# crowsonkb/style_transfer

Hardware: AMD Instinct MI355X
Metric: tile-iterations/sec, VGG-19 2048px/1024-tile (fwd+bwd, Gram/content losses, regularizers, Adam step) (higher is better)
Workload: dtype f32 (fp16x2-split MFMA, fp32 accumulate)

## Files before the change

### style_transfer_amd/csrc/common.h

```cpp
#pragma once

#include <hip/hip_runtime.h>

#include <vector>

#include <cstdarg>
#include <cstdio>
#include <functional>
#include <string>

#include "stx.h"

namespace stx {

constexpr float kEps = 1.1920928955078125e-07f;

void set_error(const char *fmt, ...);

const char *sw_env(const char *name);
void sw_reread();

#define STX_HIP(call)                                                                       \
    do {                                                                                    \
        hipError_t err__ = (call);                                                          \
// ... 120 lines not shown
    bool pin_mask = false;
#ifdef STX_EXPERIMENT_BF3
    const void *x_split = nullptr;
#endif
};

enum class ConvFamily { Direct, Wino2, H2 };

struct ConvConfig {
    ConvFamily family;
    int id;
    int bm;
    int kc;
    int pr, pc;
    int threads;
    size_t lds_bytes;
};

ConvConfig conv_pick_config(int ksize, int K, int M, int H, int W);
ConvConfig conv_config_by_id(int id);
bool direct_takes_inject(const ConvConfig &cfg);
int conv_num_workgroups(const ConvConfig &cfg, int M, int H, int W);
size_t conv_packed_floats(const ConvConfig &cfg, int K, int M, int ksize);
int conv_pack_weights(hipStream_t s, const float *w_caffe, int Mo, int Ko, int ksize,
                      int transpose_flip, const ConvConfig &cfg, float *packed);
int conv_launch(hipStream_t s, const ConvConfig &cfg, const ConvProblem &p, bool packed_weights);
int direct_splitk_factor(const ConvConfig &cfg, const ConvProblem &p, bool packed_weights);

int splitk_reduce_launch(hipStream_t s, const ConvProblem &p, int ksplit);
int splitk_reduce_items_launch(hipStream_t s, const ConvProblem &p, const ConvConfig &cfg, int slices,
                               int item_base, int items);
__host__ __device__ inline void wino2_item_tiles(int lt, int m_tiles, int n_patches, int &pt, int &mt) {
    pt = lt / m_tiles;
    mt = lt - pt * m_tiles;
    if (m_tiles == 8 && (n_patches & 7) == 0) {
        const int g = lt >> 5, r = lt & 31;
        mt = (g & 1) * 4 + (r & 3);
        pt = (g >> 1) * 8 + (r >> 2);
    }
}

struct WinoArgs {
    const float *x;
    const float *w;
    float *y;
    const float *bias;
    const float *mask;
    int K, M, H, W;
    int n_chunks, tiles_x, tiles_y, m_tiles, ksplit;
    int w_tile_stride;
    int x_bytes, w_bytes;
    int relu;
    ConvInject inj;
    float *pool_out;
    int pool_mode;
    unsigned char *pool_codes;
    int skip_y = 0;
    unsigned char *out_codes = nullptr;
    unsigned char *in_codes = nullptr;
    const unsigned char *mask_codes = nullptr;
    long long *clock_out = nullptr;
    int item_base = 0;
    const unsigned *x_amax = nullptr;
    unsigned *y_amax = nullptr;
    const unsigned char *pin_codes = nullptr;
    int pin_mode = 0, pin_mask = 0;
#ifdef STX_EXPERIMENT_BF3
    int vp_rows = 0, vp_tp = 0;
#endif
};

bool conv_first_usable(int K, int M, int ksize);
int conv_first_workgroups(int H, int W);
int conv_first_launch(hipStream_t s, const float *x, const float *w_caffe, const float *bias, float *y,
                      int K, int H, int W, int relu, float *gram_partials, unsigned *y_amax = nullptr);

ConvConfig wino2_config(int geometry = 0);
int wino2_pick_geometry(int H, int W);
size_t wino2_packed_floats(int K, int M);
int wino2_pack_weights(hipStream_t s, const float *w_caffe, int Mo, int Ko, int transpose_flip,
                       float *packed);
int wino2_launch(hipStream_t s, const ConvConfig &cfg, const ConvProblem &p, int ksplit);
bool wino2_fuses_pool(const ConvProblem &p);
bool wino2_uses_relu_codes(const ConvProblem &p, int ksplit);
bool wino2_writes_out_codes(const ConvConfig &cfg, const ConvProblem &p);
int wino2_splitk_factor(const ConvConfig &cfg, const ConvProblem &p);
struct Wino2Tail { int items, slices; };
Wino2Tail wino2_tail_split(const ConvConfig &cfg, const ConvProblem &p);
int wino2_max_slices(const ConvConfig &cfg, const ConvProblem &p);

constexpr int kAmaxSlots = 64;
ConvConfig h2_config(int mb, int pb = 1);
ConvConfig h2_pick_config(const ConvProblem &p);
bool h2_usable(const ConvProblem &p);
size_t h2_packed_floats(int K, int M);
int h2_pack_weights(hipStream_t s, const float *w_caffe, int Mo, int Ko, int transpose_flip, float *packed);
int h2_launch(hipStream_t s, const ConvConfig &cfg, const ConvProblem &p, int ksplit);
int h2_splitk_factor(const ConvConfig &cfg, const ConvProblem &p);
bool h2_fuses_pool(const ConvProblem &p);
bool h2_takes_pooled_input(const ConvConfig &cfg, const ConvProblem &p);
int absmax_launch(hipStream_t s, const float *x, size_t n, unsigned *slots);

size_t conv_small_packed_floats(int K);
int conv_small_pack(hipStream_t s, const float *w_caffe, int Mo, int Ko, int transpose_flip,
                    float *packed);
int conv_small_launch(hipStream_t s, const float *x, const float *packed, float *y,
                      const float *mask, int K, int M, int H, int W);

bool conv_h2_enabled();
struct ConvTuner { int device; hipStream_t stream; hipEvent_t ev0, ev1; std::function<int(const ConvConfig &, const float **)> bank; };
int conv_choose(const ConvProblem &p, bool winograd, const ConvTuner *tuner, ConvConfig *out);
struct ConvBank { int key; size_t floats; std::function<int(hipStream_t, const float *w_caffe, float *packed)> pack; };
ConvBank conv_bank(const ConvConfig &cfg, int dir, int Mo, int Ko, int ksize);
ConvBank conv_small_bank(int Mo, int Ko);
int conv_dispatch(hipStream_t s, const ConvConfig &cfg, const ConvProblem &p, double *flop_algorithmic,
                  double *flop_issued);
int conv_splitk_factor(const ConvConfig &cfg, const ConvProblem &p);
size_t conv_splitk_floats(const ConvConfig &cfg, const ConvProblem &p);
bool conv_takes_clock(const ConvConfig &cfg);
bool conv_fuses_pool(const ConvConfig &cfg, const ConvProblem &p);
bool conv_writes_pool_codes(const ConvConfig &cfg);
bool conv_reads_x_amax(const ConvConfig &cfg);
bool conv_leaves_y_amax(const ConvConfig &cfg);
bool conv_takes_inject(const ConvConfig &cfg);
bool conv_takes_pooled_input(const ConvConfig &cfg, const ConvProblem &p);
bool conv_uses_relu_codes(const ConvConfig &cfg, const ConvProblem &p, int ksplit);
bool conv_writes_out_codes(const ConvConfig &cfg, const ConvProblem &p, int ksplit);

int pool_forward_launch(hipStream_t s, const float *x, int C, int H, int W, int mode, float *y,
                        unsigned char *codes = nullptr);
int pool_backward_codes_launch(hipStream_t s, const float *dy, const unsigned char *codes, int C,
                               int H, int W, int mode, bool relu_mask, float *dx);
int pool_backward_launch(hipStream_t s, const float *dy, const float *x, int C, int H, int W,
                         int mode, bool relu_mask, float *dx);

struct GramPlan {
    int C, HW, splits, tiles;
    int parts;
    size_t partial_floats;
};
GramPlan gram_plan(int C, int HW);
bool gram_h2_usable(const float *feat, int C, int HW);
int gram_partials_launch(hipStream_t s, const float *feat, const GramPlan &plan, float *partials,
                         const unsigned *f_amax = nullptr);
int gram_finish_blocks(const GramPlan &plan);
int gram_finish_launch(hipStream_t s, const float *partials, const GramPlan &plan, float *gram_out,
                       const float *target, float *dsym, float *sumsq, unsigned short *pieces = nullptr,
                       const unsigned *f_amax = nullptr, float *block_out = nullptr);

size_t symm_pieces_elems(int C);
int symm_num_workgroups(int C, int HW);
bool symm_bf3_usable(const float *feat, const float *out, int C, int HW);
bool symm_h2_usable(const float *feat, const float *out, int C, int HW);
int symm_h2_launch(hipStream_t s, const float *feat, const float *dsym, const unsigned *d_amax, int n_damax,
                   const unsigned *f_amax, float *out, float *partials, int C, int HW);
int symm_bf3_launch(hipStream_t s, const float *feat, const float *dsym, unsigned short *pieces,
                    bool pieces_ready, float *out, float *partials, int C, int HW);

#ifdef __HIPCC__
__device__ __forceinline__ int content_origin_y(const ContentWindow &w) { return w.oy - w.sy; }
__device__ __forceinline__ int content_origin_x(const ContentWindow &w) { return w.ox - w.sx; }
__device__ __forceinline__ size_t content_index(const ContentWindow &w, int c, int y, int x) {
    int yy = (content_origin_y(w) + y) % w.ch;
    int xx = (content_origin_x(w) + x) % w.cw;
    if (yy < 0) yy += w.ch;
    if (xx < 0) xx += w.cw;
    return ((size_t)c * w.ch + yy) * w.cw + xx;
}
#endif

struct SumJob {
    const float *src;
    int n;
    float *dst;
};
int sum_jobs_launch(hipStream_t s, const SumJob *jobs, int n_jobs);
int content_sums_launch(hipStream_t s, const float *feat, const float *content,
                        const ContentWindow &win, float *sums , std::vector<SumJob> *defer = nullptr);
int inject_style_launch(hipStream_t s, float *diff, const float *sgrad, size_t n,
                        const float *abs_sum, float coef, bool accumulate, unsigned *y_amax = nullptr);
int inject_content_launch(hipStream_t s, float *diff, const float *feat, const float *content,
                          const ContentWindow &win, const float *sums, float coef, bool accumulate,
                          unsigned *y_amax = nullptr);
int relu_inplace_launch(hipStream_t s, float *x, size_t n);
int sum_partials_launch(hipStream_t s, const float *partials, int n, float *out);
int sum_partials2_launch(hipStream_t s, const float *a, int na, float *out_a, const float *b, int nb,
                         float *out_b);

constexpr int kMaskParts = 1024;
constexpr int kMaskSgradParts = 2048;
int mask_map_launch(hipStream_t s, const float *mask, int H, int W, int scale, float *out);
int mask_apply_launch(hipStream_t s, const float *feat, const float *map, const ContentWindow &win, float *fm,
                      float *m2_partials, int *n_parts);
int mask_target_launch(hipStream_t s, const float *gs, int C, const float *m2_partials, int n_parts, int HW,
                       float *out, float *a_out);
int mask_sgrad_launch(hipStream_t s, float *sgrad, const float *map, const ContentWindow &win, const float *a,
                      float *partials, int *n_parts);

constexpr int kContentMaskParts = 1024;
int content_mask_mean_launch(hipStream_t s, const float *map, const ContentWindow &win, float *a_out);
int content_mask_term_launch(hipStream_t s, const float *feat, const float *content, const float *map,
                             const ContentWindow &win, const float *a, float *sgrad, float *partials,
                             int *n_parts);

constexpr int kStatSlice = 16384;
constexpr float kStatEps = 1e-5f;
int stat_slices(int HW);
size_t stat_scratch_floats(int C, int HW);
int stat_partials_launch(hipStream_t s, const float *feat, int C, int HW, float *partials);
int stat_finish_launch(hipStream_t s, const float *partials, int C, int HW, const float *MU, const float *SD,
                       float *table, float *e_out, float *mean_out, float *sd_out);
int stat_grad_launch(hipStream_t s, const float *feat, int C, int HW, const float *table, float *sgrad,
                     float *abs_partials, int *n_parts);

int cut_tile_launch(hipStream_t s, const float *img, int H, int W, int rx, int ry, int y0, int x0,
                    int th, int tw, float *tile);
int put_tile_launch(hipStream_t s, float *grad, int H, int W, int rx, int ry, int y0, int x0,
                    int th, int tw, const float *tile);
int place_window_launch(hipStream_t s, float *dst, int dh, int dw, int y0, int x0, const float *src,
                        int C, int h, int w);
int roll_add_launch(hipStream_t s, float *acc, const float *src, int C, int h, int w, int sx, int sy,
                    float alpha, bool init);
int resample_launch(hipStream_t s, int axis, const float *src, int C, int H, int W, float *dst,
                    int OH, int OW, const int *bounds, const double *k, int ksize, int clamp);
int finish_partials_launch(hipStream_t s, const float *partials, int n, double *out_dev);
int finish_partials_n_launch(hipStream_t s, const float *partials, int n, int nv, double *out_dev);
int regularizers_launch(hipStream_t s, const float *img, float *grad, int H, int W,
                        const float mean[3], float tv_scale, float tv_power, float p_scale,
                        float p_power, const float *aux, float aux_scale, int aux_rx, int aux_ry,
                        double *loss_terms , float *scratch, size_t scratch_floats);

int swt_padded_side(int H, int W);
int swt_haar_launch(hipStream_t s, const float *img, float *grad, int H, int W, int rx, int ry,
                    float scale, float power, double *loss_term, float *scratch,
                    size_t scratch_floats);
void swt_levels_scratch(int H, int W, size_t *tmp_floats, size_t *partial_floats);
int swt_haar_levels_launch(hipStream_t s, const float *img, float *grad, int H, int W, int levels,
                           int rx, int ry, float scale, float power, double *loss_term, float *tmp,
                           float *partials);
void swt_daub_table(int order, int levels, int N, std::vector<float> *taps, int *hl);
int swt_table_launch(hipStream_t s, const float *img, float *grad, int H, int W, const float *table,
                     int ntaps, int hl, int rx, int ry, float scale, float power,
                     double *loss_term, float *tmp, float *partials);

constexpr int kLapMaxPools = 4;
struct LapLevels {
    int n;
    int lp[kLapMaxPools], hp[kLapMaxPools], wp[kLapMaxPools], off[kLapMaxPools];
};
size_t lap_levels(int H, int W, int n_pools, const int *pools, LapLevels *lv);
size_t lap_scratch_floats(size_t map_floats);
int lap_target_launch(hipStream_t s, const float *content, int H, int W, const LapLevels &lv,
                      float *target, float *scratch);
int lap_launch(hipStream_t s, const float *img, float *grad, int H, int W, const LapLevels &lv,
               size_t map_floats, const float *coefs, const float *target, double *loss_terms,
               float *scratch);

int adam_launch(hipStream_t s, float *params, const float *grad, float *g1, float *g2, float *p1,
                float *avg, size_t n, double lr, double b1, double b2, double bp1, double c1,
                double c2, double cp);
int dot_launch(hipStream_t s, const float *x, const float *y, size_t n, double *out_dev,
               float *scratch, size_t scratch_floats);
int abs_sum_launch(hipStream_t s, const float *x, size_t n, double *out_dev, float *scratch,
                   size_t scratch_floats);
int axpy_launch(hipStream_t s, float a, const float *x, float *y, size_t n);
int scale_launch(hipStream_t s, float a, float *x, size_t n);
int axpy_dev_launch(hipStream_t s, double c1, const double *a, double da, double c2, const double *b,
                    double db, const float *x, float *y, size_t n);
int scale_dev_launch(hipStream_t s, double c, const double *den, double den_div, float *x, size_t n);
int axpy_dot_dev_launch(hipStream_t s, double c1, const double *a, double da, double c2, const double *b,
                        double db, double c_s, const double *den_s, double div_s, const float *x,
                        const float *src, float *y, const float *z, size_t n, double *out_dev, float *scratch,
                        size_t scratch_floats);
int lbfgs_pair_launch(hipStream_t s, const float *g_new, float *g_old, const float *sv, float *y, size_t n,
                      double *out_dev2, float *scratch, size_t scratch_floats);
int scale2_axpy_launch(hipStream_t s, float c1, float c2, float *sv, float *params, size_t n);
int step_stats_launch(hipStream_t s, const float *avg, float *old, int H, int W,
                      double *out_dev , float *scratch, size_t scratch_floats);
int to_u8_launch(hipStream_t s, const float *img, int H, int W, const float mean[3], uint8_t *out);
int to_u8_luma_launch(hipStream_t s, const float *img, const float *content, int H, int W,
                      const float mean[3], uint8_t *out);
int color_stats_launch(hipStream_t s, const float *img, int H, int W, double *out_dev ,
                       float *scratch, size_t scratch_floats);
int color_affine_launch(hipStream_t s, const float *src, float *dst, int H, int W, const double A[9],
                        const double b[3], const float mean[3]);

}
```

### style_transfer_amd/csrc/symm.hip

```cpp

#include <algorithm>
#include <cstdlib>
#include <cstring>

#include "bf16x3.h"
#include "common.h"
#include "f16x2.h"

#ifndef STX_SYMM_SKIP
#define STX_SYMM_SKIP 0
#endif

namespace stx {

namespace {

constexpr int kSM = 64;
constexpr int kSN = 256;
#ifndef STX_SYMM_KSK
#define STX_SYMM_KSK 32
#endif
constexpr int kSK = STX_SYMM_KSK;
constexpr int kSPC = kSK / 16;
constexpr int kSegs = kSK / 8;
// ... 213 lines not shown
    const __amdgpu_buffer_rsrc_t rd =
        __builtin_amdgcn_make_buffer_rsrc(const_cast<float *>(D), 0, (unsigned)(C * C) * 4u, 0x00020000);
    unsigned voff[2];
#pragma unroll
    for (int j = 0; j < 2; ++j) {
        const int px = px0 + j * 32 + l31;
        voff[j] = px < HW ? (unsigned)((g * 8) * HW + px) * 4u : kOob;
    }
    const unsigned HW4 = (unsigned)HW * 4u;
    const int n_steps = Cp / 16, n_chunks = Cp / kSK;

    unsigned dvoff[kHDLoads], ddst[kHDLoads];
    int dcol[kHDLoads];
#pragma unroll
    for (int n = 0; n < kHDLoads; ++n) {
        const int e = tid + 256 * n;
        const int row = e / (kSK / 4), seg = e - row * (kSK / 4);
        dcol[n] = seg * 4;
        dvoff[n] = m0 + row < C ? (unsigned)((m0 + row) * C + seg * 4) * 4u : kOob;
        ddst[n] = (unsigned)(row * kRowBytes + seg * 8);
    }
    u32x4y dreg[kHDLoads];
    auto d_load = [&](int chunk) {
        const unsigned so = (unsigned)__builtin_amdgcn_readfirstlane(chunk * kSK * 4);
#pragma unroll
        for (int n = 0; n < kHDLoads; ++n)
            dreg[n] = __builtin_amdgcn_raw_buffer_load_b128(rd, dcol[n] + chunk * kSK < C ? dvoff[n] : kOob, so, 0);
    };

    float raw[kRing][2][8];
    auto f_load = [&](int step, int slot_) {
        const int k0 = __builtin_amdgcn_readfirstlane(step * 16);
        const int left = C - k0 < 16 ? C - k0 : 16;
        const __amdgpu_buffer_rsrc_t rk =
            BIG ? __builtin_amdgcn_make_buffer_rsrc(const_cast<float *>(F) + (size_t)k0 * (size_t)HW, 0,
                                                    (left > 0 ? left : 0) * HW * 4, 0x00020000)
                : rf;
#pragma unroll
        for (int j = 0; j < 2; ++j)
#pragma unroll
            for (int e = 0; e < 8; ++e)
                raw[slot_][j][e] = __builtin_bit_cast(
                    float, __builtin_amdgcn_raw_buffer_load_b32(
                               rk, voff[j], BIG ? (unsigned)e * HW4 : (unsigned)min(k0 + e, C) * HW4, 0));
    };

    f32x16h acc[2][2];
#pragma unroll
    for (int i = 0; i < 2; ++i)
#pragma unroll
        for (int j = 0; j < 2; ++j)
#pragma unroll
            for (int r = 0; r < 16; ++r) acc[i][j][r] = 0.f;

    d_load(0);
#pragma unroll
    for (int r = 0; r < kRing - 1; ++r)
        if (r < n_steps) f_load(r, r);

    const int ef = h2_scale_exp(amax_of_slots(f_amax, kAmaxSlots));
    unsigned dm = 0;
    for (int i = tid; i < n_damax; i += 256) dm = max(dm, d_amax[i]);
#pragma unroll
    for (int off = 32; off > 0; off >>= 1) dm = max(dm, (unsigned)__shfl_xor((int)dm, off, 64));
    if (lane == 0) wave_max[wave] = dm;
    __syncthreads();
    dm = max(max(wave_max[0], wave_max[1]), max(wave_max[2], wave_max[3]));
    const int ed = __builtin_amdgcn_readfirstlane(h2_scale_exp(dm));
    const float sf = pow2f(ef), sd = pow2f(ed);

    auto d_store = [&](int buf) {
#pragma unroll
        for (int n = 0; n < kHDLoads; ++n) {
            unsigned h[2], l[2];
            const unsigned d0 = dreg[n].x, d1 = dreg[n].y, d2 = dreg[n].z, d3 = dreg[n].w;
            split2_f16_quad(__builtin_bit_cast(float, d0), __builtin_bit_cast(float, d1),
                            __builtin_bit_cast(float, d2), __builtin_bit_cast(float, d3), sd, h, l);
            typedef unsigned u32x2s __attribute__((ext_vector_type(2)));
            unsigned char *q = lds + buf * kHChunkBytes + ddst[n];
            *reinterpret_cast<u32x2s *>(q) = (u32x2s){h[0], h[1]};
            *reinterpret_cast<u32x2s *>(q + kPieceBytes) = (u32x2s){l[0], l[1]};
        }
    };
    d_store(0);
    if (n_chunks > 1) d_load(1);
    __syncthreads();

    const unsigned a_off = (unsigned)(l31 * kRowBytes + g * 16);
    auto do_step = [&](int slot_, int buf, int s_in_chunk) {
        f16x8h bh[2], bl[2], ah[2], al[2];
#pragma unroll
        for (int j = 0; j < 2; ++j) split2_f16(raw[slot_][j], sf, bh[j], bl[j]);
        const unsigned char *base = lds + buf * kHChunkBytes + a_off + s_in_chunk * 32;
#pragma unroll
        for (int i = 0; i < 2; ++i) {
            ah[i] = *reinterpret_cast<const f16x8h *>(base + i * 32 * kRowBytes);
            al[i] = *reinterpret_cast<const f16x8h *>(base + kPieceBytes + i * 32 * kRowBytes);
        }
#pragma unroll
        for (int i = 0; i < 2; ++i)
#pragma unroll
            for (int j = 0; j < 2; ++j) acc[i][j] = mfma_split3(ah[i], al[i], bh[j], bl[j], acc[i][j]);
    };

    int step = 0;
    auto advance = [&](int slot_) {
        const int chunk = step / kSPC, s_in = step % kSPC, buf = chunk & 1;
        if (step + kRing - 1 < n_steps) f_load(step + kRing - 1, (slot_ + kRing - 1) % kRing);
        do_step(slot_, buf, s_in);
        if (s_in == kSPC - 1) {
            if (chunk + 1 < n_chunks) d_store(buf ^ 1);
            if (chunk + 2 < n_chunks) d_load(chunk + 2);
            __syncthreads();
        }
        ++step;
    };
    while (step < n_steps) {
#pragma unroll
        for (int r = 0; r < kRing; ++r)
            if (step < n_steps) advance(r);
    }

    const float ud = pow2f(-ed), uf = pow2f(-ef);
    float asum = 0.f;
#pragma unroll
    for (int i = 0; i < 2; ++i)
#pragma unroll
        for (int r = 0; r < 16; ++r) {
            const int row = m0 + i * 32 + (r & 3) + 8 * (r >> 2) + 4 * g;
            const int row0 = min(__builtin_amdgcn_readfirstlane(m0 + i * 32 + (r & 3) + 8 * (r >> 2)), C);
            const unsigned so = BIG ? 0u : (unsigned)row0 * HW4;
            const int rows_left = C - row0 < 5 ? C - row0 : 5;
            const __amdgpu_buffer_rsrc_t rrow =
                BIG ? __builtin_amdgcn_make_buffer_rsrc(S + (size_t)row0 * (size_t)HW, 0,
                                                        (rows_left > 0 ? rows_left : 0) * HW * 4, 0x00020000)
                    : rs;
#pragma unroll
            for (int j = 0; j < 2; ++j) {
                const int px = px0 + j * 32 + l31;
                const bool ok = row < C && px < HW;
                const float v = (acc[i][j][r] * ud) * uf;
                asum += ok ? fabsf(v) : 0.f;
                const unsigned vo = ok ? (unsigned)((4 * g) * HW + px) * 4u : kOob;
                __builtin_amdgcn_raw_buffer_store_b32(__builtin_bit_cast(unsigned, v), rrow, vo, so, 0);
            }
        }
#pragma unroll
    for (int off = 32; off > 0; off >>= 1) asum += __shfl_down(asum, off, 64);
    if (lane == 0) wave_sum[wave] = asum;
    __syncthreads();
    if (tid == 0) partials[blockIdx.x] = ((wave_sum[0] + wave_sum[1]) + wave_sum[2]) + wave_sum[3];
}

__global__ void symm_split_kernel(const float *__restrict__ dsym, int C, int Cp,
                                  unsigned short *__restrict__ pieces) {
    const int idx = blockIdx.x * blockDim.x + threadIdx.x;
    if (idx >= Cp * Cp) return;
    const int i = idx / Cp, j = idx - i * Cp;
    unsigned short s1 = 0, s2 = 0, s3 = 0;
    if (i < C && j < C) split3_bf16_scalar(dsym[i * C + j], s1, s2, s3);
    pieces[idx] = s1;
    pieces[(size_t)Cp * Cp + idx] = s2;
    pieces[2 * (size_t)Cp * Cp + idx] = s3;
}

int symm_num_workgroups(int C, int HW) { return ceil_div(C, kSM) * ceil_div(HW, kSN); }

bool symm_bf3_usable(const float *feat, const float *out, int C, int HW) {
    const char *env = sw_env("STX_SYMM");
    if (env && !strcmp(env, "fp32")) return false;
    return 64.0 * (double)HW < 2147483648.0 &&
           ((reinterpret_cast<uintptr_t>(feat) | reinterpret_cast<uintptr_t>(out)) & 3) == 0;
}

int symm_bf3_launch(hipStream_t s, const float *feat, const float *dsym, unsigned short *pieces,
                    bool pieces_ready, float *out, float *partials, int C, int HW) {
    const int Cp = ceil_div(C, kSM) * kSM;
    if (!pieces_ready || Cp != C) {
        symm_split_kernel<<<ceil_div(Cp * Cp, 256), 256, 0, s>>>(dsym, C, Cp, pieces);
        STX_CHECK_LAUNCH();
    }
    const int m_tiles = Cp / kSM;
    const double bytes = 4.0 * C * (double)HW;
    const char *force_big = sw_env("STX_WINO_BIG");
    if (bytes >= 2147483648.0 || (force_big && atoi(force_big) == 1))
        symm_bf3_kernel<true><<<symm_num_workgroups(C, HW), 256, 0, s>>>(feat, pieces, out, partials, C, Cp,
                                                                       HW, 0u, m_tiles);
    else
        symm_bf3_kernel<false><<<symm_num_workgroups(C, HW), 256, 0, s>>>(feat, pieces, out, partials, C, Cp,
                                                                        HW, (unsigned)bytes, m_tiles);
    STX_CHECK_LAUNCH();
    return STX_OK;
}

bool symm_h2_usable(const float *feat, const float *out, int C, int HW) {
    const char *env = sw_env("STX_SYMM");
    if (env && (!strcmp(env, "fp32") || !strcmp(env, "bf3"))) return false;
    return C % 4 == 0 && symm_bf3_usable(feat, out, C, HW);
}

int symm_h2_launch(hipStream_t s, const float *feat, const float *dsym, const unsigned *d_amax, int n_damax,
                   const unsigned *f_amax, float *out, float *partials, int C, int HW) {
    const int Cp = ceil_div(C, kSM) * kSM;
    const int m_tiles = Cp / kSM;
    const double bytes = 4.0 * C * (double)HW;
    const char *force_big = sw_env("STX_WINO_BIG");
    if (bytes >= 2147483648.0 || (force_big && atoi(force_big) == 1))
        symm_h2_kernel<true><<<symm_num_workgroups(C, HW), 256, 0, s>>>(feat, dsym, d_amax, n_damax, f_amax, out,
                                                                      partials, C, Cp, HW, 0u, m_tiles);
    else
        symm_h2_kernel<false><<<symm_num_workgroups(C, HW), 256, 0, s>>>(feat, dsym, d_amax, n_damax, f_amax, out,
                                                                       partials, C, Cp, HW, (unsigned)bytes, m_tiles);
    STX_CHECK_LAUNCH();
    return STX_OK;
}

}
```

### style_transfer_amd/csrc/tile_path.cpp

```cpp

#include <algorithm>
#include <cmath>
#include <cstdlib>
#include <deque>

#include "engine.h"

namespace stx {

ConvProblem conv_fwd_problem(const float *x, float *y, const float *bias, int Cin, int Cout, int H, int W,
                             int ks, int relu) {
    ConvProblem p{};
    p.x = x;
    p.y = y;
    p.bias = bias;
    p.K = Cin;
    p.M = Cout;
    p.H = H;
    p.W = W;
    p.ksize = ks;
    p.relu = relu;
    p.epilogue = kEpiForward;
    return p;
}
// ... 206 lines not shown
        p.pool_out = pt.data.f();
        p.pool_mode = pool->pool_mode;
        pt.codes_valid = false;
        pt.amax_data = -1;
        if (conv_fuses_pool(cfg, p)) {
            *pooled = true;
            pt.amax_data = t.amax_data;
            if (conv_writes_pool_codes(cfg) && e->pool_codes) {
                STX_TRY(pt.codes.ensure(pt.count() + 4));
                p.pool_codes = static_cast<unsigned char *>(pt.codes.ptr);
                pt.codes_valid = true;
                p.skip_y = plan.top_unobserved;
            }
        } else {
            p.pool_out = nullptr;
        }
    }
    t.relu_codes_valid = false;
    if (plan.relu_codes && t.relu && plan.conv_reader && conv_h2_enabled()) {
        const size_t bytes = (size_t)t.channels * ((t.h + 1) / 2) * ((t.w + 1) / 2);
        STX_TRY(t.relu_codes.ensure(bytes));
        p.out_codes = static_cast<unsigned char *>(t.relu_codes.ptr);
        t.relu_codes_valid = conv_writes_out_codes(cfg, p, conv_splitk_factor(cfg, p));
        if (!t.relu_codes_valid) p.out_codes = nullptr;
    }
    ProfScope scope(e, "fwd " + L.name, direct);
    return launch_conv(e, cfg, p);
}

static ConvProblem conv_backward_shape(stx_engine *e, int li) {
    const Layer &L = e->layers[li];
    const Blob &b = e->blobs[L.bottom_blob];
    const ConvParams &cp = e->sh->conv[li];
    return conv_bwd_problem(nullptr, nullptr, nullptr, cp.cout, cp.cin, b.h, b.w, cp.ks);
}

static bool conv_backward_takes_pooled(stx_engine *e, int li) {
    const char *env = sw_env("STX_POOL_BWD_FUSE");
    if (env && atoi(env) == 0) return false;
    const ConvProblem p = conv_backward_shape(e, li);
    ConvConfig cfg;
    return p.ksize == 3 && p.M > 4 && conv_choose(p, e->winograd, nullptr, &cfg) == STX_OK &&
           conv_takes_pooled_input(cfg, p);
}

static int run_conv_backward(stx_engine *e, int li, const ConvInject *inj, bool *fused, const Layer *pooled) {
    const Layer &L = e->layers[li];
    Blob &b = e->blobs[L.bottom_blob];
    const Blob &t = e->blobs[L.top_blob];
    const ConvParams &cp = e->sh->conv[li];
    ConvProblem p = conv_backward_shape(e, li);
    p.x = t.diff.f();
    p.y = b.diff.f();
    p.mask = b.relu ? b.data.f() : nullptr;
    p.mask_codes = b.relu && b.relu_codes_valid ? static_cast<const unsigned char *>(b.relu_codes.ptr) : nullptr;
    p.wants_codes = b.relu && b.relu_codes_wanted;
    if (cp.ks == 3 && cp.cin <= 4) {
        if (fused) *fused = false;
        const float *packed = nullptr;
        STX_TRY(get_bank(e, li, conv_small_bank(cp.cout, cp.cin), &packed));
        const double direct = conv_flops(cp.cout, cp.cin, b.h, b.w, cp.ks);
        ProfScope scope(e, "bwd " + L.name, direct);
        e->flop_algorithmic += direct;
        e->flop_issued += direct * 4.0 / p.M;
        return conv_small_launch(e->stream, p.x, packed, p.y, p.mask, p.K, p.M, p.H, p.W);
    }
    ConvConfig cfg;
    STX_TRY(choose_conv(e, li, 1, p, &cfg));
    const bool can_fuse = inj && conv_takes_inject(cfg);
    if (fused) *fused = can_fuse;
    if (can_fuse) p.inject = *inj;
    b.amax_diff = -1;
    if (pooled) {
        const Blob &pt = e->blobs[pooled->top_blob];
        if (!conv_takes_pooled_input(cfg, p) || !pt.codes_valid) {
            set_error("run_conv_backward: %s cannot take the gradient of %s pooled", L.name.c_str(), pt.name.c_str());
            return STX_ERR_UNSUPPORTED;
        }
        p.x = pt.diff.f();
        p.pin_codes = static_cast<const unsigned char *>(pt.codes.ptr);
        p.pin_mode = pooled->pool_mode;
        p.pin_mask = t.relu;
        STX_TRY(amax_for(e, pooled->top_blob, true, &p.x_amax));
    } else if (conv_reads_x_amax(cfg)) {
        STX_TRY(amax_for(e, L.top_blob, true, &p.x_amax));
    }
    if (conv_leaves_y_amax(cfg)) {
        p.y_amax = e->amax_slots(L.bottom_blob, true);
        b.amax_diff = L.bottom_blob;
    }
    STX_TRY(get_packed(e, li, 1, cfg, &p.w));
    STX_TRY(attach_splitk(e, cfg, p));
    ProfScope scope(e, "bwd " + L.name, conv_flops(cp.cout, cp.cin, b.h, b.w, cp.ks));
    return launch_conv(e, cfg, p);
}

static size_t style_term_scratch_floats(int C, int HW) {
    return 2 * (size_t)ceil_div(C * C, 64) + (size_t)symm_num_workgroups(C, HW) + 64;
}

int launch_style_terms(stx_engine *e, hipStream_t stream, const float *feat, int C, int h, int w,
                       const float *target, float *sgrad, float *sc, const std::string &name,
                       const unsigned *f_amax, float *term_scratch, std::vector<SumJob> *defer) {
    const int HW = h * w;
    const bool fused = e->first_gram_valid && e->first_gram_blob >= 0 &&
                       feat == e->blobs[e->first_gram_blob].data.f() && C == 64;
    GramPlan plan = gram_plan(C, HW);
    if (fused) {
        plan.splits = e->first_gram_parts;
        plan.tiles = 1;
        plan.parts = 1;
        plan.partial_floats = (size_t)plan.splits * 64 * 64;
    }
    const int fin_blocks = gram_finish_blocks(plan);
    float *const partials = fused ? e->first_gram.f() : nullptr;
    if (!fused) STX_TRY(e->gram_partials.ensure((plan.partial_floats + 2 * fin_blocks) * sizeof(float)));
    STX_TRY(e->dsym.ensure((size_t)C * C * sizeof(float)));
    const bool gram_h2 = !fused && gram_h2_usable(feat, C, HW);
    const bool symm_h2 = symm_h2_usable(feat, sgrad, C, HW);
    const bool bf3 = !symm_h2 && symm_bf3_usable(feat, sgrad, C, HW);
    if ((gram_h2 || symm_h2) && !f_amax) {
        unsigned *scratch;
        STX_TRY(amax_scratch(e, &scratch));
        ProfScope scope(e, "absmax " + name, 0.0, stream);
        STX_TRY(absmax_launch(stream, feat, (size_t)C * HW, scratch));
        f_amax = scratch;
    }
    if (bf3) STX_TRY(e->dsym_pieces.ensure(symm_pieces_elems(C) * sizeof(unsigned short)));
    unsigned short *pieces = bf3 && C % 64 == 0 ? static_cast<unsigned short *>(e->dsym_pieces.ptr) : nullptr;
    {
        ProfScope scope(e, "gram " + name, 2.0 * C * C * (double)HW, stream);
        if (!fused) STX_TRY(gram_partials_launch(stream, feat, plan, e->gram_partials.f(), gram_h2 ? f_amax : nullptr));
        STX_TRY(gram_finish_launch(stream, fused ? partials : e->gram_partials.f(), plan, nullptr, target,
                                   e->dsym.f(), nullptr, pieces, gram_h2 ? f_amax : nullptr,
                                   defer ? term_scratch : nullptr));
    }
    ProfScope scope(e, "symm " + name, 2.0 * C * C * (double)HW, stream);
    const float *block_sumsq = defer ? term_scratch : (fused ? partials : e->gram_partials.f()) + plan.partial_floats;
    auto finish = [&](float *symm_partials, int n_wg) -> int {
        if (!defer) return sum_partials2_launch(stream, block_sumsq, fin_blocks, sc, symm_partials, n_wg, sc + 1);
        defer->push_back(SumJob{block_sumsq, fin_blocks, sc});
        defer->push_back(SumJob{symm_partials, n_wg, sc + 1});
        return STX_OK;
    };
    if (symm_h2 || bf3) {
        const int n_wg = symm_num_workgroups(C, HW);
        float *symm_partials = defer ? term_scratch + 2 * fin_blocks : nullptr;
        if (!defer) {
            STX_TRY(e->symm_partials.ensure((size_t)n_wg * sizeof(float)));
            symm_partials = e->symm_partials.f();
        }
        if (symm_h2)
            STX_TRY(symm_h2_launch(stream, feat, e->dsym.f(), reinterpret_cast<const unsigned *>(block_sumsq + fin_blocks),
                                   fin_blocks, f_amax, sgrad, symm_partials, C, HW));
        else
            STX_TRY(symm_bf3_launch(stream, feat, e->dsym.f(), static_cast<unsigned short *>(e->dsym_pieces.ptr),
                                    pieces != nullptr, sgrad, symm_partials, C, HW));
        return finish(symm_partials, n_wg);
    }
    const ConvConfig cfg = conv_pick_config(1, C, C, h, w);
    const int n_wg = conv_num_workgroups(cfg, C, h, w);
    STX_TRY(e->symm_partials.ensure((size_t)n_wg * sizeof(float)));
    ConvProblem p{};
    p.x = feat;
    p.w = e->dsym.f();
    p.y = sgrad;
    p.partials = e->symm_partials.f();
    p.K = C;
    p.M = C;
    p.H = h;
    p.W = w;
    p.ksize = 1;
    p.epilogue = kEpiSymm;
    STX_TRY(conv_launch(stream, cfg, p, false));
    return sum_partials2_launch(stream, block_sumsq, fin_blocks, sc, e->symm_partials.f(), n_wg, sc + 1);
}

int launch_masked_style_terms(stx_engine *e, hipStream_t stream, const float *feat, int C, int h, int w,
                              const float *mask_map, const ContentWindow &win, const float *target,
                              float *sgrad, float *sc, const std::string &name, const unsigned *f_amax,
                              float *term_scratch, float *mask_scratch, std::vector<SumJob> *defer) {
    STX_TRY(e->masked_feat.ensure((size_t)C * h * w * sizeof(float)));
    STX_TRY(e->masked_target.ensure((size_t)C * C * sizeof(float)));
    float *const m2_partials = mask_scratch, *const ms_partials = mask_scratch + kMaskParts;
    {
        ProfScope scope(e, "mask " + name, 0.0, stream);
        int n_m2 = 0;
        STX_TRY(mask_apply_launch(stream, feat, mask_map, win, e->masked_feat.f(), m2_partials, &n_m2));
        STX_TRY(mask_target_launch(stream, target, C, m2_partials, n_m2, h * w, e->masked_target.f(), sc + 3));
    }
    STX_TRY(launch_style_terms(e, stream, e->masked_feat.f(), C, h, w, e->masked_target.f(), sgrad, sc, name,
                               f_amax, term_scratch, defer));
    ProfScope scope(e, "smask " + name, 0.0, stream);
    int n_ms = 0;
    STX_TRY(mask_sgrad_launch(stream, sgrad, mask_map, win, sc + 3, ms_partials, &n_ms));
    if (!defer) return sum_partials_launch(stream, ms_partials, n_ms, sc + 2);
    defer->push_back(SumJob{ms_partials, n_ms, sc + 2});
    return STX_OK;
}

int launch_stat_terms(stx_engine *e, hipStream_t stream, const float *feat, int C, int h, int w, const float *MU,
                      const float *SD, float *sgrad, float *sc, const std::string &name, float *stat_scratch,
                      std::vector<SumJob> *defer) {
    const int HW = h * w;
    float *const partials = stat_scratch;
    float *const table = partials + 4 * (size_t)C * stat_slices(HW);
    float *const abs_partials = table + 4 * (size_t)C;
    ProfScope scope(e, "stat " + name, 0.0, stream);
    STX_TRY(stat_partials_launch(stream, feat, C, HW, partials));
    STX_TRY(stat_finish_launch(stream, partials, C, HW, MU, SD, table, sc, nullptr, nullptr));
    int n_parts = 0;
    STX_TRY(stat_grad_launch(stream, feat, C, HW, table, sgrad, abs_partials, &n_parts));
    if (!defer) return sum_partials_launch(stream, abs_partials, n_parts, sc + 1);
    defer->push_back(SumJob{abs_partials, n_parts, sc + 1});
    return STX_OK;
}

int launch_masked_content_terms(stx_engine *e, hipStream_t stream, const float *feat, const float *content,
                                const float *mask_map, const ContentWindow &win, float *sgrad, float *sc,
                                const std::string &name, float *partials, std::vector<SumJob> *defer) {
    ProfScope scope(e, "cmask " + name, 0.0, stream);
    STX_TRY(content_mask_mean_launch(stream, mask_map, win, sc + 2));
    int n = 0;
    STX_TRY(content_mask_term_launch(stream, feat, content, mask_map, win, sc + 2, sgrad, partials, &n));
    if (!defer) return sum_partials2_launch(stream, partials, n, sc, partials + n, n, sc + 1);
    defer->push_back(SumJob{partials, n, sc});
    defer->push_back(SumJob{partials + n, n, sc + 1});
    return STX_OK;
}

static int begin_timing(stx_engine *e) {
    e->ev_cur = (e->ev_cur + 1) % stx_engine::kTimed;
    STX_HIP(hipEventRecord(e->ev_start[e->ev_cur], e->stream));
    e->flop_algorithmic = e->flop_issued = 0;
    return STX_OK;
}

static int end_timing(stx_engine *e) {
    STX_HIP(hipEventRecord(e->ev_stop[e->ev_cur], e->stream));
    if (e->ev_recorded < stx_engine::kTimed) ++e->ev_recorded;
    e->timed = true;
    return STX_OK;
}

namespace {

struct Tap {
    int blob;
    const stx_tap *t;
};

struct TileCall {
    const float *img;
    int img_mem, th, tw, rx, ry, start[2];
    const stx_tap *taps;
    int n_taps;
    float *grad_out;
    int grad_mem;
};

struct TilePlan {
    std::vector<Tap> order;
    std::vector<char> needed;
    std::vector<int> tap_of;
    std::deque<stx_tap> extra;
};

struct Term {
    bool style;
    const float *src;
    const float *sums;
    float coef;
    ContentWindow win;
};

struct TileRun {
    stx_engine *e;
    const TileCall &c;
    const TilePlan &plan;
    PendingLoss &pl;
    bool sums_late;
    bool interleave;
    std::vector<std::vector<Term>> terms;
    std::vector<SumJob> sum_jobs;
    size_t scratch_used;
    std::vector<SumJob> *defer() { return sums_late ? &sum_jobs : nullptr; }
};

}

static const StatTarget *stat_target_of(const stx_engine *e, int blob) {
    for (const StatTarget &t : e->sh->stats)
        if (t.blob == blob) return &t;
    return nullptr;
}

static int sc_grad_prepare(stx_engine *e, const TileCall &c, TilePlan &plan) {
    std::vector<Tap> &order = plan.order;
    const stx_tap *taps = c.taps;
    const int n_taps = c.n_taps;
    for (int i = 0; i < n_taps; ++i) {
        const int blob = e->find_blob(taps[i].layer);
        if (blob <= 0) {
            set_error("stx_sc_grad_tile: unknown tap layer '%s'",
                      taps[i].layer ? taps[i].layer : "(null)");
            return STX_ERR_ARG;
        }
// ... 622 lines not shown
```

Before: 267.3.

## Add 128-row symm h2 kernel to reuse feature loads across two M tiles

Adds a variant of the fp16x2-split symm kernel in which each workgroup computes 128 output rows instead of 64. Each feature-map load and split is then reused for two D row tiles, which halves global F traffic and the split work. Partial sums are written into the same slots the 64-row layout would use, so the downstream reductions do not change. It is chosen by default when the paired grid still has at least 512 workgroups. The trade-off is more accumulator registers and LDS per workgroup, with launch bounds set to 2 workgroups per CU.

```diff
diff --git a/style_transfer_amd/csrc/common.h b/style_transfer_amd/csrc/common.h
--- a/style_transfer_amd/csrc/common.h
+++ b/style_transfer_amd/csrc/common.h
@@ -296,8 +296,9 @@
 int symm_num_workgroups(int C, int HW);
 bool symm_bf3_usable(const float *feat, const float *out, int C, int HW);
 bool symm_h2_usable(const float *feat, const float *out, int C, int HW);
+bool symm_rows128_wanted(int C, int HW);
 int symm_h2_launch(hipStream_t s, const float *feat, const float *dsym, const unsigned *d_amax, int n_damax,
-                   const unsigned *f_amax, float *out, float *partials, int C, int HW);
+                   const unsigned *f_amax, float *out, float *partials, int C, int HW, bool rows128 = false);
 int symm_bf3_launch(hipStream_t s, const float *feat, const float *dsym, unsigned short *pieces,
                     bool pieces_ready, float *out, float *partials, int C, int HW);
 
diff --git a/style_transfer_amd/csrc/symm.hip b/style_transfer_amd/csrc/symm.hip
--- a/style_transfer_amd/csrc/symm.hip
+++ b/style_transfer_amd/csrc/symm.hip
@@ -389,6 +389,192 @@
     if (tid == 0) partials[blockIdx.x] = ((wave_sum[0] + wave_sum[1]) + wave_sum[2]) + wave_sum[3];
 }
 
+constexpr int kSM2 = 2 * kSM;
+constexpr int kPieceBytes2 = kSM2 * kRowBytes;
+constexpr int kHChunkBytes2 = 2 * kPieceBytes2;
+constexpr int kHDLoads2 = kSM2 * kSK / 4 / 256;
+
+__global__ __launch_bounds__(256, 2) void symm_h2_rows128_kernel(const float *__restrict__ F,
+                                                                 const float *__restrict__ D,
+                                                                 const unsigned *__restrict__ d_amax, int n_damax,
+                                                                 const unsigned *__restrict__ f_amax,
+                                                                 float *__restrict__ S,
+                                                                 float *__restrict__ partials, int C, int Cp,
+                                                                 int HW, unsigned f_bytes, int m_tiles, int m_pairs) {
+    __shared__ __attribute__((aligned(16))) unsigned char lds[2 * kHChunkBytes2];
+    __shared__ float wave_sum[2][4];
+    __shared__ unsigned wave_max[4];
+    const int tid = threadIdx.x, lane = tid & 63;
+    const int wave = __builtin_amdgcn_readfirstlane(tid >> 6);
+    const int l31 = lane & 31, g = lane >> 5;
+    const int nb = gridDim.x, xcd = blockIdx.x & 7, slot = blockIdx.x >> 3;
+    const int q8 = nb >> 3, r8 = nb & 7;
+    const int L = (xcd < r8 ? xcd * (q8 + 1) : r8 * (q8 + 1) + (xcd - r8) * q8) + slot;
+    const int mp = __builtin_amdgcn_readfirstlane(L % m_pairs), pt = __builtin_amdgcn_readfirstlane(L / m_pairs);
+    const int m0 = mp * kSM2;
+    const bool two = 2 * mp + 1 < m_tiles;
+    const int px0 = pt * kSN + wave * 64;
+
+    constexpr unsigned kOob = 0x80000000u;
+    const __amdgpu_buffer_rsrc_t rf = __builtin_amdgcn_make_buffer_rsrc(const_cast<float *>(F), 0, f_bytes, 0x00020000);
+    const __amdgpu_buffer_rsrc_t rs = __builtin_amdgcn_make_buffer_rsrc(S, 0, f_bytes, 0x00020000);
+    const __amdgpu_buffer_rsrc_t rd =
+        __builtin_amdgcn_make_buffer_rsrc(const_cast<float *>(D), 0, (unsigned)(C * C) * 4u, 0x00020000);
+    unsigned voff[2];
+#pragma unroll
+    for (int j = 0; j < 2; ++j) {
+        const int px = px0 + j * 32 + l31;
+        voff[j] = px < HW ? (unsigned)((g * 8) * HW + px) * 4u : kOob;
+    }
+    const unsigned HW4 = (unsigned)HW * 4u;
+    const int n_steps = Cp / 16, n_chunks = Cp / kSK;
+
+    unsigned dvoff[kHDLoads2], ddst[kHDLoads2];
+    int dcol[kHDLoads2];
+#pragma unroll
+    for (int n = 0; n < kHDLoads2; ++n) {
+        const int e = tid + 256 * n;
+        const int row = e / (kSK / 4), seg = e - row * (kSK / 4);
+        dcol[n] = seg * 4;
+        dvoff[n] = m0 + row < C ? (unsigned)((m0 + row) * C + seg * 4) * 4u : kOob;
+        ddst[n] = (unsigned)(row * kRowBytes + seg * 8);
+    }
+    u32x4y dreg[kHDLoads2];
+    auto d_load = [&](int chunk) {
+        const unsigned so = (unsigned)__builtin_amdgcn_readfirstlane(chunk * kSK * 4);
+#pragma unroll
+        for (int n = 0; n < kHDLoads2; ++n)
+            dreg[n] = __builtin_amdgcn_raw_buffer_load_b128(rd, dcol[n] + chunk * kSK < C ? dvoff[n] : kOob, so, 0);
+    };
+
+    float raw[kRing][2][8];
+    auto f_load = [&](int step, int slot_) {
+        const int k0 = __builtin_amdgcn_readfirstlane(step * 16);
+#pragma unroll
+        for (int j = 0; j < 2; ++j)
+#pragma unroll
+            for (int e = 0; e < 8; ++e)
+                raw[slot_][j][e] = __builtin_bit_cast(
+                    float, __builtin_amdgcn_raw_buffer_load_b32(rf, voff[j], (unsigned)min(k0 + e, C) * HW4, 0));
+    };
+
+    f32x16h acc[4][2];
+#pragma unroll
+    for (int i = 0; i < 4; ++i)
+#pragma unroll
+        for (int j = 0; j < 2; ++j)
+#pragma unroll
+            for (int r = 0; r < 16; ++r) acc[i][j][r] = 0.f;
+
+    d_load(0);
+#pragma unroll
+    for (int r = 0; r < kRing - 1; ++r)
+        if (r < n_steps) f_load(r, r);
+
+    const int ef = h2_scale_exp(amax_of_slots(f_amax, kAmaxSlots));
+    unsigned dm = 0;
+    for (int i = tid; i < n_damax; i += 256) dm = max(dm, d_amax[i]);
+#pragma unroll
+    for (int off = 32; off > 0; off >>= 1) dm = max(dm, (unsigned)__shfl_xor((int)dm, off, 64));
+    if (lane == 0) wave_max[wave] = dm;
+    __syncthreads();
+    dm = max(max(wave_max[0], wave_max[1]), max(wave_max[2], wave_max[3]));
+    const int ed = __builtin_amdgcn_readfirstlane(h2_scale_exp(dm));
+    const float sf = pow2f(ef), sd = pow2f(ed);
+
+    auto d_store = [&](int buf) {
+#pragma unroll
+        for (int n = 0; n < kHDLoads2; ++n) {
+            unsigned h[2], l[2];
+            const unsigned d0 = dreg[n].x, d1 = dreg[n].y, d2 = dreg[n].z, d3 = dreg[n].w;
+            split2_f16_quad(__builtin_bit_cast(float, d0), __builtin_bit_cast(float, d1),
+                            __builtin_bit_cast(float, d2), __builtin_bit_cast(float, d3), sd, h, l);
+            typedef unsigned u32x2s __attribute__((ext_vector_type(2)));
+            unsigned char *q = lds + buf * kHChunkBytes2 + ddst[n];
+            *reinterpret_cast<u32x2s *>(q) = (u32x2s){h[0], h[1]};
+            *reinterpret_cast<u32x2s *>(q + kPieceBytes2) = (u32x2s){l[0], l[1]};
+        }
+    };
+    d_store(0);
+    if (n_chunks > 1) d_load(1);
+    __syncthreads();
+
+    const unsigned a_off = (unsigned)(l31 * kRowBytes + g * 16);
+    auto do_step = [&](int slot_, int buf, int s_in_chunk) {
+        f16x8h bh[2], bl[2];
+#pragma unroll
+        for (int j = 0; j < 2; ++j) split2_f16(raw[slot_][j], sf, bh[j], bl[j]);
+        const unsigned char *base = lds + buf * kHChunkBytes2 + a_off + s_in_chunk * 32;
+#pragma unroll
+        for (int i = 0; i < 4; ++i) {
+            if (i >= 2 && !two) continue;
+            const f16x8h ah = *reinterpret_cast<const f16x8h *>(base + i * 32 * kRowBytes);
+            const f16x8h al = *reinterpret_cast<const f16x8h *>(base + kPieceBytes2 + i * 32 * kRowBytes);
+#pragma unroll
+            for (int j = 0; j < 2; ++j) acc[i][j] = mfma_split3(ah, al, bh[j], bl[j], acc[i][j]);
+        }
+    };
+
+    int step = 0;
+    auto advance = [&](int slot_) {
+        const int chunk = step / kSPC, s_in = step % kSPC, buf = chunk & 1;
+        if (step + kRing - 1 < n_steps) f_load(step + kRing - 1, (slot_ + kRing - 1) % kRing);
+        do_step(slot_, buf, s_in);
+        if (s_in == kSPC - 1) {
+            if (chunk + 1 < n_chunks) d_store(buf ^ 1);
+            if (chunk + 2 < n_chunks) d_load(chunk + 2);
+            __syncthreads();
+        }
+        ++step;
+    };
+    while (step < n_steps) {
+#pragma unroll
+        for (int r = 0; r < kRing; ++r)
+            if (step < n_steps) advance(r);
+    }
+
+    const float ud = pow2f(-ed), uf = pow2f(-ef);
+    float asum[2] = {0.f, 0.f};
+#pragma unroll
+    for (int i = 0; i < 4; ++i) {
+        if (i >= 2 && !two) continue;
+#pragma unroll
+        for (int r = 0; r < 16; ++r) {
+            const int row = m0 + i * 32 + (r & 3) + 8 * (r >> 2) + 4 * g;
+            const int row0 = min(__builtin_amdgcn_readfirstlane(m0 + i * 32 + (r & 3) + 8 * (r >> 2)), C);
+            const unsigned so = (unsigned)row0 * HW4;
+#pragma unroll
+            for (int j = 0; j < 2; ++j) {
+                const int px = px0 + j * 32 + l31;
+                const bool ok = row < C && px < HW;
+                const float v = (acc[i][j][r] * ud) * uf;
+                asum[i >> 1] += ok ? fabsf(v) : 0.f;
+                const unsigned vo = ok ? (unsigned)((4 * g) * HW + px) * 4u : kOob;
+                __builtin_amdgcn_raw_buffer_store_b32(__builtin_bit_cast(unsigned, v), rs, vo, so, 0);
+            }
+        }
+    }
+#pragma unroll
+    for (int h = 0; h < 2; ++h) {
+#pragma unroll
+        for (int off = 32; off > 0; off >>= 1) asum[h] += __shfl_down(asum[h], off, 64);
+        if (lane == 0) wave_sum[h][wave] = asum[h];
+    }
+    __syncthreads();
+    if (tid < 2 && (tid == 0 || two)) {
+        const int nb1 = m_tiles * (nb / m_pairs), q1 = nb1 >> 3, r1 = nb1 & 7;
+        const int L1 = pt * m_tiles + 2 * mp + tid;
+        int x1, s1;
+        if (L1 < r1 * (q1 + 1)) {
+            x1 = L1 / (q1 + 1), s1 = L1 - x1 * (q1 + 1);
+        } else {
+            const int rest = L1 - r1 * (q1 + 1);
+            x1 = r1 + rest / q1, s1 = rest - (rest / q1) * q1;
+        }
+        partials[s1 * 8 + x1] = ((wave_sum[tid][0] + wave_sum[tid][1]) + wave_sum[tid][2]) + wave_sum[tid][3];
+    }
+}
+
 __global__ void symm_split_kernel(const float *__restrict__ dsym, int C, int Cp,
                                   unsigned short *__restrict__ pieces) {
     const int idx = blockIdx.x * blockDim.x + threadIdx.x;
@@ -436,13 +622,29 @@
     return C % 4 == 0 && symm_bf3_usable(feat, out, C, HW);
 }
 
+bool symm_rows128_wanted(int C, int HW) {
+    if (C < kSM2) return false;
+    const char *env = sw_env("STX_SYMM_ROWS");
+    if (env && atoi(env) == 64) return false;
+    if (env && atoi(env) == 128) return true;
+    return ceil_div(ceil_div(C, kSM), 2) * ceil_div(HW, kSN) >= 512;
+}
+
 int symm_h2_launch(hipStream_t s, const float *feat, const float *dsym, const unsigned *d_amax, int n_damax,
-                   const unsigned *f_amax, float *out, float *partials, int C, int HW) {
+                   const unsigned *f_amax, float *out, float *partials, int C, int HW, bool rows128) {
     const int Cp = ceil_div(C, kSM) * kSM;
     const int m_tiles = Cp / kSM;
     const double bytes = 4.0 * C * (double)HW;
     const char *force_big = sw_env("STX_WINO_BIG");
-    if (bytes >= 2147483648.0 || (force_big && atoi(force_big) == 1))
+    const bool big = bytes >= 2147483648.0 || (force_big && atoi(force_big) == 1);
+    if (rows128 && !big && m_tiles >= 2) {
+        const int m_pairs = ceil_div(m_tiles, 2);
+        symm_h2_rows128_kernel<<<m_pairs * ceil_div(HW, kSN), 256, 0, s>>>(
+            feat, dsym, d_amax, n_damax, f_amax, out, partials, C, Cp, HW, (unsigned)bytes, m_tiles, m_pairs);
+        STX_CHECK_LAUNCH();
+        return STX_OK;
+    }
+    if (big)
         symm_h2_kernel<true><<<symm_num_workgroups(C, HW), 256, 0, s>>>(feat, dsym, d_amax, n_damax, f_amax, out,
                                                                       partials, C, Cp, HW, 0u, m_tiles);
     else
diff --git a/style_transfer_amd/csrc/tile_path.cpp b/style_transfer_amd/csrc/tile_path.cpp
--- a/style_transfer_amd/csrc/tile_path.cpp
+++ b/style_transfer_amd/csrc/tile_path.cpp
@@ -382,7 +382,7 @@
         }
         if (symm_h2)
             STX_TRY(symm_h2_launch(stream, feat, e->dsym.f(), reinterpret_cast<const unsigned *>(block_sumsq + fin_blocks),
-                                   fin_blocks, f_amax, sgrad, symm_partials, C, HW));
+                                   fin_blocks, f_amax, sgrad, symm_partials, C, HW, symm_rows128_wanted(C, HW)));
         else
             STX_TRY(symm_bf3_launch(stream, feat, e->dsym.f(), static_cast<unsigned short *>(e->dsym_pieces.ptr),
                                     pieces != nullptr, sgrad, symm_partials, C, HW));
```

Result: no change. 267.2 (-0.0%).
